# hahnyuan/PTQ4ViT

Hardware: AMD Instinct MI355X
Metric: calibration throughput (wrapped modules calibrated per second), ViT-B/224 W8A8, 32 calibration images (higher is better)
Workload: dtype int8

## Files before the change

include/ptq4vit_hip_debug.h:

```cpp
#ifndef PTQ4VIT_HIP_DEBUG_H
#define PTQ4VIT_HIP_DEBUG_H

#include <stddef.h>
#include <stdint.h>

#ifdef __cplusplus
extern "C" {
#endif

int p4v_debug_set_variant(int variant, int force_generic);
int p4v_debug_set_tuning(int key, int value);
int p4v_debug_bound_totals(float* out, int64_t capacity, int64_t* count);
int p4v_debug_set_arena_gap(size_t bytes);
int p4v_debug_arena_ranges(uint64_t* out, int cap);
int p4v_debug_mlp_planes(uint64_t* out);
int p4v_debug_attn_planes(uint64_t info[5]);
int p4v_debug_sos_sweep(const p4v_matmul_desc* desc, const float* d_A, const float* d_B, const float* d_out, const float* d_grad,
                        int n_cands, int c_lo, int c_hi, int known_cands, float* d_scores, void* d_workspace, size_t workspace_bytes,
                        void* stream);
int p4v_debug_topk_rows(const float* d_mass, int segs, int n, int k, int32_t* d_idx, void* stream);
int p4v_debug_pack_dual(const float* d_x, long rows, long cols, long cols_padded, int sos, int lo, int hi, int qmax,
                        const float* d_scale, float const_scale, int8_t* d_q1, int8_t* d_q2, void* stream);
int p4v_debug_pack_cands(const float* d_x, long rows, long cols, long rows_padded, long cols_padded, int layout, int lo, int hi,
                         const float* d_scales, int n_cands, const int* d_crange, const unsigned char* d_done, int live_max,
                         int general, int8_t* d_q, void* stream);
int p4v_debug_gather_im2col(int batch, int in_channels, int height, int width, int kernel_h, int kernel_w, int stride_h, int stride_w,
                            int pad_h, int pad_w, int dil_h, int dil_w, const float* d_x, const int32_t* d_idx, int k, float* d_dst,
                            void* stream);
int p4v_debug_prep_epi6(const float* d_o, const float* d_wt, const float* d_bias, long o_ss, long o_ts, int sr, int tr,
                        int bias_on_t, int wt_mode, int transposed, float* d_e, void* stream);

#ifdef __cplusplus
}
#endif
#endif
```

ptq4vit_amd/_lib.py:

```python
import ctypes as C
import os

_HERE = os.path.dirname(os.path.abspath(__file__))
LIB_PATH = os.environ.get("P4V_LIB") or os.path.join(_HERE, "csrc", "libptq4vit_hip.so")

METRICS = {
    "L1_norm": 0,
    "L2_norm": 1,
    "linear_weighted_L2_norm": 2,
    "square_weighted_L2_norm": 3,
    "hessian": 4,
    "cosine": 5,
}


class LinearDesc(C.Structure):
    _fields_ = [(n, C.c_int32) for n in (
        "batch", "tokens", "in_features", "out_features", "n_V", "n_H", "n_a", "w_bit", "a_bit", "metric",
        "eq_n", "search_round", "twin_postgelu", "init_layerwise", "has_bias", "reserved")]


class MlpDesc(C.Structure):
    _fields_ = [("fc1", LinearDesc), ("fc2", LinearDesc)]

# ... 63 lines not shown

JOB_LINEAR, JOB_MATMUL, JOB_CONV, JOB_MATMUL_BLOCKS = 0, 1, 2, 3
RESERVED_FP32_PLANES, RESERVED_NO_MEMO, RESERVED_FORWARD_ONLY, RESERVED_NO_PRUNE = 1, 2, 4, 8
RESERVED_BLOCK_SHIFT = 8


def reserved_block(block):
    return 0 if block is None else (int(block) + 1) << RESERVED_BLOCK_SHIFT


PLANE_SYM, PLANE_SOS_HI, PLANE_SOS_LO, PLANE_TWIN = 1, 2, 3, 4
EXPORT_SYM_I8, EXPORT_SYM_F32, EXPORT_GELU_U8, EXPORT_SOS_U8 = 0, 1, 2, 3


EXPORTS = [
    "p4v_version", "p4v_last_error",
    "p4v_linear_workspace_bytes", "p4v_linear_calibrate",
    "p4v_matmul_workspace_bytes", "p4v_matmul_calibrate",
    "p4v_matmul_blocks_workspace_bytes", "p4v_matmul_blocks_calibrate", "p4v_amax_init_matmul_blocks",
    "p4v_matmul_blocks_search", "p4v_matmul_blocks_quant_forward",
    "p4v_conv_workspace_bytes", "p4v_conv_calibrate",
    "p4v_calibrate_group", "p4v_launch_counters",
    "p4v_linear_quant_forward", "p4v_matmul_quant_forward", "p4v_mlp_workspace_bytes", "p4v_mlp_quant_forward",
    "p4v_attn_workspace_bytes", "p4v_attn_quant_forward",
    "p4v_amax_init_linear", "p4v_linear_search_w", "p4v_linear_search_a",
    "p4v_amax_init_matmul", "p4v_matmul_search_A", "p4v_sos_search_split", "p4v_matmul_search_B",
    "p4v_amax_init_conv", "p4v_conv_search_w_channelwise", "p4v_conv_search_w_layerwise", "p4v_conv_search_a",
    "p4v_score_argmax_gather",
    "p4v_quantize_i8", "p4v_pack_plane_i8", "p4v_fake_quant", "p4v_export_quantize", "p4v_multi_copy",
    "p4v_stats_enable", "p4v_stats_reset", "p4v_stats_get", "p4v_stats_launches", "p4v_prune_counters",
    "p4v_debug_set_variant", "p4v_debug_set_tuning", "p4v_debug_bound_totals", "p4v_debug_topk_rows", "p4v_debug_pack_dual", "p4v_debug_prep_epi6",
    "p4v_debug_pack_cands", "p4v_debug_gather_im2col", "p4v_debug_sos_sweep",
    "p4v_debug_set_arena_gap", "p4v_debug_arena_ranges", "p4v_debug_mlp_planes", "p4v_debug_attn_planes",
]

_lib = None


def load():
    global _lib
    if _lib is not None:
        return _lib
    if not os.path.exists(LIB_PATH):
        raise RuntimeError(
            f"ptq4vit_amd: HIP extension {LIB_PATH} is missing -- build it with "
            "`python -c 'import __graft_entry__ as g; g.build()'` (hipcc --offload-arch=gfx950). "
            "There is no CPU fallback for the calibration path.")
    import torch
    lib = C.CDLL(LIB_PATH)
    vp, fp, ip = C.c_void_p, C.c_void_p, C.c_void_p
    lib.p4v_version.restype = C.c_int
    lib.p4v_last_error.restype = C.c_char_p
    lib.p4v_linear_workspace_bytes.restype = C.c_size_t
    lib.p4v_linear_workspace_bytes.argtypes = [C.POINTER(LinearDesc)]
    lib.p4v_linear_calibrate.restype = C.c_int
    lib.p4v_linear_calibrate.argtypes = [C.POINTER(LinearDesc), fp, fp, fp, fp, fp, fp, fp, fp, fp, ip, vp, C.c_size_t, vp]
    lib.p4v_matmul_workspace_bytes.restype = C.c_size_t
    lib.p4v_matmul_workspace_bytes.argtypes = [C.POINTER(MatMulDesc)]
    lib.p4v_matmul_calibrate.restype = C.c_int
    lib.p4v_matmul_calibrate.argtypes = [C.POINTER(MatMulDesc), fp, fp, fp, fp, fp, fp, fp, fp, fp, ip, vp, C.c_size_t, vp]
    MBD = C.POINTER(MatMulBlocksDesc)
    lib.p4v_matmul_blocks_workspace_bytes.restype = C.c_size_t
    lib.p4v_matmul_blocks_workspace_bytes.argtypes = [MBD]
    lib.p4v_matmul_blocks_calibrate.restype = C.c_int
    lib.p4v_matmul_blocks_calibrate.argtypes = [MBD, fp, fp, fp, fp, fp, fp, fp, fp, fp, ip, vp, C.c_size_t, vp]
    lib.p4v_amax_init_matmul_blocks.restype = C.c_int
# ... 23 lines not shown
    lib.p4v_matmul_quant_forward.restype = C.c_int
    lib.p4v_matmul_quant_forward.argtypes = [C.POINTER(MatMulDesc), fp, fp, fp, fp, fp, fp, vp, C.c_size_t, vp]
    LD, MD, CD = C.POINTER(LinearDesc), C.POINTER(MatMulDesc), C.POINTER(ConvDesc)
    tail = [vp, C.c_size_t, vp]
    for name, args in (
            ("p4v_amax_init_linear", [LD] + [fp] * 4),
            ("p4v_linear_search_w", [LD] + [fp] * 9 + [ip]),
            ("p4v_linear_search_a", [LD] + [fp] * 9 + [ip]),
            ("p4v_amax_init_matmul", [MD] + [fp] * 4),
            ("p4v_matmul_search_A", [MD] + [fp] * 8 + [ip]),
            ("p4v_sos_search_split", [MD] + [fp] * 7 + [ip]),
            ("p4v_matmul_search_B", [MD] + [fp] * 9 + [ip]),
            ("p4v_amax_init_conv", [CD] + [fp] * 4),
            ("p4v_conv_search_w_channelwise", [CD] + [fp] * 9 + [ip]),
            ("p4v_conv_search_w_layerwise", [CD] + [fp] * 9 + [ip]),
            ("p4v_conv_search_a", [CD] + [fp] * 9 + [ip])):
        fn = getattr(lib, name)
        fn.restype = C.c_int
        fn.argtypes = args + tail
    lib.p4v_score_argmax_gather.restype = C.c_int
    lib.p4v_score_argmax_gather.argtypes = [fp, C.c_int32, C.c_int32, fp, fp, ip, vp]
    lib.p4v_quantize_i8.restype = C.c_int
    lib.p4v_quantize_i8.argtypes = [fp, C.c_int64, C.c_int64, C.c_int64, fp, C.c_int64, C.c_int32, C.c_int32, vp, vp]
    lib.p4v_fake_quant.restype = C.c_int
    lib.p4v_fake_quant.argtypes = [fp, C.c_int64, C.c_int64, fp, C.c_int64, C.c_int32, C.c_int32, fp, vp]
    lib.p4v_pack_plane_i8.restype = C.c_int
    lib.p4v_pack_plane_i8.argtypes = [C.POINTER(PlaneDesc), fp, fp, vp, vp]
    lib.p4v_export_quantize.restype = C.c_int
    lib.p4v_export_quantize.argtypes = [C.POINTER(ExportDesc), fp, fp, fp, vp, vp]
    lib.p4v_multi_copy.restype = C.c_int
    lib.p4v_multi_copy.argtypes = [vp, C.c_int32, C.c_int64, C.c_int64, vp]
    lib.p4v_debug_topk_rows.restype = C.c_int
    lib.p4v_debug_topk_rows.argtypes = [vp, C.c_int, C.c_int, C.c_int, vp, vp]
    lib.p4v_debug_pack_dual.restype = C.c_int
    lib.p4v_debug_pack_dual.argtypes = [fp, C.c_long, C.c_long, C.c_long, C.c_int, C.c_int, C.c_int, C.c_int, fp, C.c_float, vp, vp, vp]
    lib.p4v_debug_pack_cands.restype = C.c_int
    lib.p4v_debug_pack_cands.argtypes = [fp, C.c_long, C.c_long, C.c_long, C.c_long, C.c_int, C.c_int, C.c_int, fp, C.c_int, vp, vp,
                                         C.c_int, C.c_int, vp, vp]
    lib.p4v_debug_gather_im2col.restype = C.c_int
    lib.p4v_debug_gather_im2col.argtypes = [C.c_int] * 12 + [fp, ip, C.c_int, fp, vp]
    lib.p4v_debug_sos_sweep.restype = C.c_int
    lib.p4v_debug_sos_sweep.argtypes = [C.POINTER(MatMulDesc), fp, fp, fp, fp, C.c_int, C.c_int, C.c_int, C.c_int, fp, vp, C.c_size_t, vp]
    lib.p4v_debug_prep_epi6.restype = C.c_int
    lib.p4v_debug_prep_epi6.argtypes = [fp, fp, fp, C.c_long, C.c_long, C.c_int, C.c_int, C.c_int, C.c_int, C.c_int, fp, vp]
    lib.p4v_debug_set_variant.restype = C.c_int
    lib.p4v_debug_set_variant.argtypes = [C.c_int, C.c_int]
    lib.p4v_debug_set_tuning.restype = C.c_int
    lib.p4v_debug_set_tuning.argtypes = [C.c_int, C.c_int]
    lib.p4v_debug_set_arena_gap.restype = C.c_int
    lib.p4v_debug_set_arena_gap.argtypes = [C.c_size_t]
    lib.p4v_debug_arena_ranges.restype = C.c_int
    lib.p4v_debug_arena_ranges.argtypes = [C.POINTER(C.c_uint64), C.c_int]
    lib.p4v_debug_bound_totals.restype = C.c_int
    lib.p4v_debug_bound_totals.argtypes = [fp, C.c_int64, C.POINTER(C.c_int64)]
    lib.p4v_stats_enable.restype = C.c_int
    lib.p4v_stats_enable.argtypes = [C.c_int]
    lib.p4v_stats_reset.restype = C.c_int
    lib.p4v_stats_get.restype = C.c_int
    lib.p4v_stats_get.argtypes = [C.POINTER(KernelStats)]
    lib.p4v_stats_launches.restype = C.c_int
    lib.p4v_stats_launches.argtypes = [C.POINTER(LaunchRecord), C.c_int64, C.POINTER(C.c_int64)]
    lib.p4v_prune_counters.restype = C.c_int
    lib.p4v_prune_counters.argtypes = [C.POINTER(C.c_int64), C.c_int]
    lib.p4v_launch_counters.restype = C.c_int
    lib.p4v_launch_counters.argtypes = [C.POINTER(C.c_int64), C.c_int]
    lib.p4v_calibrate_group.restype = C.c_int
# ... 22 lines not shown
```

ptq4vit_amd/csrc/p4v_api.hip:

```cpp
#include <hip/hip_runtime.h>

#include <algorithm>
#include <atomic>
#include <climits>
#include <cstdarg>
#include <cstdio>
#include <condition_variable>
#include <cstring>
#include <deque>
#include <functional>
#include <thread>
#include <mutex>
#include <string>
#include <unordered_map>
#include <type_traits>
#include <vector>

#include "../../include/ptq4vit_hip.h"
#include "../../include/ptq4vit_hip_debug.h"
#include "p4v_kernels.h"

using namespace p4v;

namespace {
// ... 429 lines not shown
    for (auto& m : g_mir) if (m.dev == dev) return &m;
    return nullptr;
}
void attach_mirror(SelectParams& sl) {
    sl.iv_host = nullptr; sl.aux_host = nullptr;
    IvMirror* mi = mirror_of(sl.interval);
    IvMirror* ma = mirror_of(sl.aux_out);
    if (mi) mi->valid = false;
    if (ma) ma->valid = false;
    if (mi && sl.nj <= MIR_SLOT && sl.out_off == 0 && (sl.nj == 1 || sl.out_js == 1)) { sl.iv_host = mi->host; mi->valid = true; mi->count = sl.nj; }
    if (ma && sl.nj <= MIR_SLOT) { sl.aux_host = ma->host; ma->valid = true; ma->count = sl.nj; }
}

void metric_epi(int metric, int* epi, int* wt_mode) {
    switch (metric) {
        case P4V_METRIC_L1_NORM: *epi = EPI_ABS; *wt_mode = 0; break;
        case P4V_METRIC_L2_NORM: *epi = EPI_SQ; *wt_mode = 0; break;
        case P4V_METRIC_LINEAR_WEIGHTED_L2: *epi = EPI_W_SQ; *wt_mode = 3; break;
        case P4V_METRIC_SQUARE_WEIGHTED_L2: *epi = EPI_SQ_W; *wt_mode = 2; break;
        case P4V_METRIC_HESSIAN: *epi = EPI_SQ_W; *wt_mode = 1; break;
        default: *epi = EPI_COS; *wt_mode = 0; break;
    }
}

int launch_absmax(Ctx& c, const float* src, const long (&st)[4], int D0, int D1, int R, int C, int nV, int nH,
                  int crb_r, int crb_c, int signed_max, unsigned* out) {
    if (c.dry) return 0;
    CHK(q_fill(c, out, 0, sizeof(unsigned) * (size_t)D1 * nV * nH));
    AbsMaxParams p{src, st[0], st[1], st[2], st[3], D0, D1, R, C, nV, nH, crb_r, crb_c, 0, signed_max, out};
    p.row_tile = std::max(1, std::min(crb_r, std::max(1, 8192 / std::max(1, std::min(crb_c, C)))));
    const int tiles_per_v = cdiv(crb_r, p.row_tile);
    dim3 grid(tiles_per_v * nV * nH, D1, D0);
    return enqueue(c, KERN(AbsMaxParams, k_absmax), grid, dim3(256), 0, p);
}

int launch_interval(Ctx& c, const unsigned* enc, int n, float denom, int broadcast, float* interval) {
    if (c.dry) return 0;
    return enqueue(c, KERN(IntervalParams, k_interval_from_max), dim3(cdiv(n, 64)), dim3(64), 0, IntervalParams{enc, n, denom, broadcast, interval});
}

int launch_cands(Ctx& c, const float* mult, const float* interval, int ncand, int nblk, float* cands) {
    if (c.dry) return 0;
    return enqueue(c, KERN(CandsParams, k_make_cands), dim3(cdiv((long)ncand * nblk, 256)), dim3(256), 0, CandsParams{mult, interval, ncand, nblk, cands});
}

int launch_scale(Ctx& c, ScaleParams p) {
    if (c.dry) return 0;
    return enqueue(c, KERN(ScaleParams, k_scale_table), dim3(cdiv((long)p.C * p.nblk, 256)), dim3(256), 0, p);
}

std::atomic<int> g_cvt_state{0};
void cvt_probe(hipStream_t stream) {
    if (g_cvt_state.load(std::memory_order_acquire) != 0) return;
    static std::mutex mu;
    std::lock_guard<std::mutex> lk(mu);
    if (g_cvt_state.load(std::memory_order_acquire) != 0) return;
    static unsigned* scratch = nullptr;
    if (!scratch && hipMalloc(&scratch, 8 * sizeof(unsigned)) != hipSuccess) { (void)hipGetLastError(); scratch = nullptr; return; }
    unsigned h[5] = {9, 9, 9, 9, 9};
    hipLaunchKernelGGL(k_probe_cvt, dim3(1), dim3(64), 0, stream, scratch);
    if (hipGetLastError() != hipSuccess || hipMemcpyAsync(h, scratch, sizeof h, hipMemcpyDeviceToHost, stream) != hipSuccess ||
        hipStreamSynchronize(stream) != hipSuccess) { (void)hipGetLastError(); return; }
    const bool sat = h[3] == 0 && h[4] == 255;
    const int st = (sat && h[0] == 0 && h[1] == 1 && h[2] == 2) ? 1 : (sat && h[0] == 1 && h[1] == 2 && (h[2] == 2 || h[2] == 3)) ? 2 : 3;
    if (tune(TUNE_PRINT) > 0) fprintf(stderr, "[p4v] v_cvt_pk_u8_f32(0.7, 1.5, 2.5, -3, 300) = %u %u %u %u %u -> mode %d\n", h[0], h[1], h[2], h[3], h[4], st);
    g_cvt_state.store(st, std::memory_order_release);
// ... 679 lines not shown

int pack_operand(Ctx& c, const Pass& ps, const SweepPlan& pl, const PassBufs& b, const Operand& op, char* buf, bool col, int c0, int nc) {
    PackParams pk = op.pk;
    pk.Rp = col ? pl.NpB : pl.Mp; pk.Kp = pl.Kp; pk.dst = buf;
    pk.Z = (col ? ps.col_zs_shared : ps.row_zs_shared) ? 1 : ps.Z;
    pk.C = op.expanded ? nc : 1;
    pk.c_inner = op.expanded ? pl.cin_exp : pl.cin_fix;
    if (op.expanded && pk.scales) pk.scales += (long)c0 * pk.sc_cs;
    if (op.expanded && ps.crange) {
        pk.crange = ps.crange; pk.c_base = c0;
        pk.done = (b.pc && b.pc->done) ? b.pc->done : nullptr;
    }
    int live_max = -1;
    if (pk.crange && ps.host_hi > ps.host_lo) live_max = std::max(0, std::min(ps.host_hi, c0 + nc) - std::max(ps.host_lo, c0));
    else if (pk.crange && ps.host_len > 0) live_max = std::min(ps.host_len, nc);
    return ps.i8 ? launch_pack<int8_t>(c, pk, live_max) : launch_pack<float>(c, pk, live_max);
}
int pack_expanded(Ctx& c, const Pass& ps, const SweepPlan& pl, const PassBufs& b, int c0, int nc) {
    PlaneCache* pc = b.pc;
    const bool packed = pc && pc->valid;
    if (ps.row.expanded && !packed) CHK(pack_operand(c, ps, pl, b, ps.row, b.row, false, c0, nc));
    if (ps.twin && ps.row2.expanded) CHK(pack_operand(c, ps, pl, b, ps.row2, b.row2, false, c0, nc));
    if (ps.col.expanded && !packed) CHK(pack_operand(c, ps, pl, b, ps.col, b.col, true, c0, nc));
    if (pc && !ps.crange && !packed) {
        pc->valid = true;
        if (!c.dry && pc->done) CHK(q_fill(c, pc->done, 1, (size_t)ps.eq_n));
    }
    return 0;
}

int prep_epilogue(Ctx& c, const Pass& ps, const SweepPlan& pl, const PassBufs& b) {
    const bool a_search = pl.a_search;
    const size_t zero_bytes = sizeof(float) * pl.zero_bias_n;
    if (pl.epi6_on && !c.dry && !(b.ec && b.ec->valid)) {
        PrepEpi6Params pe{};
        pe.O = ps.O; pe.Wt = ps.G ? ps.G : ps.O; pe.bias = ps.bias ? ps.bias : b.zero_bias;
        pe.o_ss = a_search ? ps.o_ns : ps.o_ms; pe.o_ts = a_search ? ps.o_ms : ps.o_ns;
        pe.SR = a_search ? ps.Ncols : ps.Mrows; pe.TR = a_search ? ps.Mrows : ps.Ncols;
        pe.bias_on_t = a_search ? 0 : 1; pe.wt_mode = ps.cos6 ? 4 : ps.wt_mode;
        pe.stiles = pl.s6_stiles; pe.ttiles = pl.s6_ttiles; pe.E = b.epi6; pe.transposed = (ps.cos6 && !a_search) ? 1 : 0;
        if (b.zero_bias) CHK(q_fill(c, b.zero_bias, 0, zero_bytes));
        CHK(enqueue(c, KERN(PrepEpi6Params, k_prep_epi6), dim3((unsigned)std::min<long>((long)pl.s6_stiles * pl.s6_ttiles, 256L * 32)), dim3(256), 0, pe));
    }
    if (b.ec) b.ec->valid = true;
    if (pl.epi7_n && !c.dry) {
        PrepEpiParams pe{ps.O, ps.G ? ps.G : ps.O, ps.bias, ps.o_ms, ps.Mrows, ps.Ncols, ps.cos7 ? 4 : ps.wt_mode,
                         pl.Np / 256, pl.Mp / (ps.twin ? 128 : 256), ps.twin ? 1 : 0, b.epi7};
        const long chunks = (long)pl.Mp * pl.Np * 2 / 4;
        CHK(enqueue(c, KERN(PrepEpiParams, k_prep_epi), dim3((unsigned)std::min<long>(cdiv(chunks, 256), 256L * 16)), dim3(256), 0, pe));
    }
    if (b.zero_bias && !c.dry) CHK(q_fill(c, b.zero_bias, 0, zero_bytes));
    return 0;
}

int pack_fixed_planes(Ctx& c, const Pass& ps, const SweepPlan& pl, const PassBufs& b) {
    if (ps.row.prepacked) {
        if (ps.row.expanded || pl.merged7 || pl.cin_fix != 0 || (ps.twin && (!ps.row2.prepacked || ps.row2.expanded)))
            return fail(P4V_ERR_INVALID, "prepacked row operand: fixed row-major plane(s) of a forward pass only");
    } else if (pl.merged7) {
        Operand both = ps.row;
        both.pk.mode = PACK_TWIN_I8;
        both.pk.lo = ps.row2.pk.lo; both.pk.neg_scale = ps.row2.pk.neg_scale;
        both.pk.dst2 = b.row2;
        CHK(pack_operand(c, ps, pl, b, both, b.row, false, 0, 1));
    } else if (ps.twin && ps.i8 && !ps.row.expanded && !ps.row2.expanded && dual_pack_ok(ps.row.pk, ps.row2.pk)) {
        PackParams p1 = ps.row.pk, p2 = ps.row2.pk;
        p1.Rp = p2.Rp = pl.Mp; p1.Kp = p2.Kp = pl.Kp; p1.Z = p2.Z = ps.row_zs_shared ? 1 : ps.Z; p1.C = p2.C = 1;
        p1.dst = b.row; p2.dst = b.row2;
        if (!c.dry) {
            const long total = (long)p1.Z * pl.Mp * (pl.Kp / 16);
            if (total >= (1L << 31)) return fail(P4V_ERR_UNSUPPORTED, "operand plane too large for k_pack_dual (%ld 16-element runs)", total);
            CHK(enqueue(c, KERN(PackDualParams, k_pack_dual), dim3((unsigned)std::min<long>(cdiv(total, 256), 256L * 64)), dim3(256), 0, PackDualParams{p1, p2}));
        }
    } else {
        if (!ps.row.expanded) CHK(pack_operand(c, ps, pl, b, ps.row, b.row, false, 0, 1));
        if (ps.twin && !ps.row2.expanded) CHK(pack_operand(c, ps, pl, b, ps.row2, b.row2, false, 0, 1));
    }
    if (!ps.col.expanded) CHK(pack_operand(c, ps, pl, b, ps.col, b.col, true, 0, 1));
    return 0;
}

int chunk_exec_frac(Ctx& c, const Pass& ps, const SweepPlan& pl, int c0, int nc) {
    g_exec_frac = 1.0;
    if (!(g_stat_on && ps.crange && !c.dry)) return 0;
// ... 213 lines not shown
    bool conv; PackParams conv_pk;
    int k_cap;
};
int slice_alloc(Ctx& c, SliceCache* sc, const SliceGeo& g, bool keep, bool bump) {
    if (sc->assigned) {
        if (sc->k != g.k_cap) return fail(P4V_ERR_INVALID, "slice cache reused with another geometry");
        return 0;
    }
    if (!keep && !bump) return 0;
    const long zrows = (long)g.segs * g.seg_rows, out_elems = (long)g.segs * g.k_cap * g.Ncols, row_elems = (long)g.segs * g.k_cap * g.K;
    if (keep) {
        sc->idx = reinterpret_cast<int*>(c.ws.get_top((size_t)g.segs * g.k_cap * sizeof(int)));
        sc->mass = reinterpret_cast<float*>(c.ws.get_top((size_t)zrows * sizeof(float)));
        sc->Os = reinterpret_cast<float*>(c.ws.get_top((size_t)out_elems * sizeof(float)));
        sc->Gs = reinterpret_cast<float*>(c.ws.get_top((size_t)out_elems * sizeof(float)));
        sc->Rs = reinterpret_cast<float*>(c.ws.get_top((size_t)row_elems * sizeof(float)));
        sc->frac = reinterpret_cast<float*>(c.ws.get_top(256));
        sc->assigned = true;
    } else {
        sc->idx = c.ws.get<int>((size_t)g.segs * g.k_cap);
        sc->mass = c.ws.get<float>((size_t)zrows);
        sc->Os = c.ws.get<float>((size_t)out_elems);
        sc->Gs = c.ws.get<float>((size_t)out_elems);
        sc->Rs = c.ws.get<float>((size_t)row_elems);
    }
    sc->k = g.k_cap;
    return 0;
}
int slice_fill(Ctx& c, SliceCache* sc, const SliceGeo& g, bool host_sync_ok) {
    const long zrows = (long)g.segs * g.seg_rows;
    const void* wsrc = g.G ? (const void*)g.G : (const void*)g.O;
    const bool new_idx = sc->idx_src != wsrc || sc->idx_wt != g.wt_mode || (g.wt_mode != 1 && sc->o_src != g.O);
    if (new_idx) {
        CHK(enqueue(c, KERN(RowMassParams, k_row_mass), dim3((unsigned)cdiv(zrows, 4)), dim3(256), 0, RowMassParams{g.G ? g.G : g.O, g.O, zrows, (long)g.Ncols, g.wt_mode, sc->mass}));
        CHK(enqueue(c, KERN(TopkParams, k_topk_rows), dim3(g.segs), dim3(1024), 0, TopkParams{sc->mass, g.seg_rows, g.k, sc->idx}));
        sc->idx_src = wsrc; sc->idx_wt = g.wt_mode;
        sc->o_src = sc->g_src = sc->r_src = nullptr;
        if (sc->frac && host_sync_ok && !(g_variant & 8388608)) {
            float f = 1.0f;
            int* hm = host_mirror(c);
            CHK(enqueue(c, KERN(MassFracParams, k_mass_fraction), dim3(1), dim3(1024), 0,
                        MassFracParams{sc->mass, zrows, sc->idx, g.segs, g.seg_rows, g.k, sc->frac, hm ? reinterpret_cast<float*>(hm + 4) : nullptr}));
            if (!hm) CHK(q_d2h(c, &f, sc->frac, sizeof f));
            CHK(q_sync(c));
            if (hm) f = *reinterpret_cast<volatile float*>(hm + 4);
            if (tune(TUNE_PRINT) > 0) fprintf(stderr, "[p4v] slice holds %.4f of the metric weight (%d x %d of %d rows)\n", f, g.segs, g.k, g.seg_rows);
            sc->frac_host = f;
            if (g.k < g.k_cap && !(f >= 0.97f)) {
                SliceGeo g2 = g;
                g2.k = g.k_cap;
                sc->idx_src = nullptr;
                return slice_fill(c, sc, g2, host_sync_ok);
            }
            const bool big_pass = zrows >= (tune(TUNE_LOOSE_ROWS) > 0 ? (long)tune(TUNE_LOOSE_ROWS) : 65536L);
            if (!(f >= (tune(TUNE_LOOSE_PCT) > 0 ? 0.01f * tune(TUNE_LOOSE_PCT) : big_pass ? 0.05f : 0.5f))) { sc->loose = true; return 0; }
        }
        sc->k_eff = g.k;
    }
    const int rows = g.segs * g.k;
    int gather_rc = 0;
    auto gather = [&](const float* src, long s0, long s3, int d3, float* dst, int seg, int zdiv, long sz2, long sz) {
        GatherParams gp{src, s0, 0, 0, s3, 1, 1, d3, sc->idx, rows, dst, seg, zdiv, sz2, sz};
        const long total = (long)rows * d3;
        if (const int r_ = enqueue(c, KERN(GatherParams, k_gather), dim3((unsigned)std::min<long>(cdiv(total, 256), 256L * 16)), dim3(256), 0, gp)) gather_rc = r_;
    };
    const int seg = g.lin ? 0 : g.k;
    const long o_seg = (long)g.seg_rows * g.Ncols;
// ... 2267 lines not shown
int p4v_debug_sos_sweep(const p4v_matmul_desc* desc, const float* d_A, const float* d_B, const float* d_out, const float* d_grad,
                        int n_cands, int c_lo, int c_hi, int known_cands, float* d_scores, void* d_workspace, size_t workspace_bytes,
                        void* stream) {
    if (!desc || !d_A || !d_B || !d_out || !d_scores || !d_workspace) return fail(P4V_ERR_INVALID, "p4v_debug_sos_sweep: null pointer");
    if (!desc->sos || n_cands < 1 || n_cands > 20 || !sos_split_ok(desc->M, desc->K, desc->N, false))
        return fail(P4V_ERR_INVALID, "p4v_debug_sos_sweep: a split-of-softmax matmul of the one-kernel split search, 1..20 candidates");
    const SosDebugSweep dbg{n_cands, c_lo, c_hi, known_cands, d_scores};
    float* d_split = nullptr;
    CHK(ws_aligned(d_workspace));
    HIPCHK(hipMalloc(&d_split, 2 * sizeof(float)));
    Ctx c = Ctx::on(stream, d_workspace, workspace_bytes);
    g_sos_debug = &dbg;
    const int rc = matmul_impl(desc, {.A = d_A, .B = d_B, .O = d_out, .G = d_grad, .A_iv = d_split + 1, .split = d_split}, Stage{ST_S1}, c);
    g_sos_debug = nullptr;
    (void)hipFree(d_split);
    return rc;
}

int p4v_debug_bound_totals(float* out, int64_t capacity, int64_t* count) {
    if (!out && !count) { g_b1_keep = true; g_b1_totals.clear(); return 0; }
    g_b1_keep = false;
    if (count) *count = (int64_t)g_b1_totals.size();
    if (out) std::copy(g_b1_totals.begin(), g_b1_totals.begin() + std::min<int64_t>(capacity, (int64_t)g_b1_totals.size()), out);
    return 0;
}

int p4v_debug_topk_rows(const float* d_mass, int segs, int n, int k, int32_t* d_idx, void* stream) {
    if (!d_mass || !d_idx || segs <= 0 || n <= 0 || k <= 0 || k > n) return fail(P4V_ERR_INVALID, "p4v_debug_topk_rows: bad argument");
    hipLaunchKernelGGL(k_topk_rows, dim3(segs), dim3(1024), 0, (hipStream_t)stream, TopkParams{d_mass, n, k, d_idx});
    HIPCHK(hipGetLastError());
    return 0;
}

int p4v_debug_pack_dual(const float* d_x, long rows, long cols, long cols_padded, int sos, int lo, int hi, int qmax,
                        const float* d_scale, float const_scale, int8_t* d_q1, int8_t* d_q2, void* stream) {
    if (!d_x || !d_scale || !d_q1 || !d_q2 || rows <= 0 || cols <= 0 || cols_padded % 64 || cols_padded < cols ||
        lo > 0 || hi < 0 || lo < -128 || hi > 127 || qmax < 2 || qmax > 128 || (!sos && !(const_scale > 0.0f)))
        return fail(P4V_ERR_INVALID, "p4v_debug_pack_dual: bad argument");
    PackParams p1 = pack2d(d_x, rows, cols, cols);
    p1.Rp = (int)rows; p1.Kp = (int)cols_padded; p1.C = 1; p1.scales = d_scale; p1.qm1 = (float)(qmax - 1);
    PackParams p2 = p1;
    p1.dst = d_q1; p2.dst = d_q2;
    if (sos) {
        p1.mode = PACK_SOS_HI; p2.mode = PACK_SOS_LO;
    } else {
        p1.lo = 0; p1.hi = hi; p2.lo = lo; p2.hi = 0; p2.scales = nullptr; p2.neg_scale = const_scale;
    }
    if (!dual_pack_ok(p1, p2)) return fail(P4V_ERR_INVALID, "p4v_debug_pack_dual: not a dual pair");
    Ctx c = Ctx::on(stream, nullptr, 0);
    const long total = rows * (cols_padded / 16);
    if (total >= (1L << 31)) return fail(P4V_ERR_UNSUPPORTED, "p4v_debug_pack_dual: plane too large");
    return enqueue(c, KERN(PackDualParams, k_pack_dual), dim3((unsigned)std::min<long>(cdiv(total, 256), 256L * 64)), dim3(256), 0,
                   PackDualParams{p1, p2});
}

int p4v_debug_pack_cands(const float* d_x, long rows, long cols, long rows_padded, long cols_padded, int layout, int lo, int hi,
                         const float* d_scales, int n_cands, const int* d_crange, const unsigned char* d_done, int live_max,
                         int general, int8_t* d_q, void* stream) {
    if (!d_x || !d_scales || !d_q || rows <= 0 || cols <= 0 || rows_padded < rows || cols_padded % 64 || cols_padded < cols ||
        layout < 0 || layout > 3 || (layout == 3 && rows_padded % 64) || lo > hi || lo < -128 || hi > 127 || n_cands <= 0 ||
        (d_done && !d_crange) || (live_max >= 0 && !d_crange))
        return fail(P4V_ERR_INVALID, "p4v_debug_pack_cands: bad argument");
    Ctx c = Ctx::on(stream, nullptr, 0);
    cvt_bias(c);
    PackParams p = pack2d(d_x, rows, cols, cols);
    p.Rp = (int)rows_padded; p.Kp = (int)cols_padded; p.dst = d_q; p.C = n_cands; p.c_inner = layout;
// ... 96 lines not shown
```

ptq4vit_amd/csrc/p4v_kernels.h:

```cpp
#pragma once
#include <hip/hip_runtime.h>
#include <stdint.h>
#include <type_traits>

namespace p4v {

typedef int v4i __attribute__((ext_vector_type(4)));
typedef int v16i __attribute__((ext_vector_type(16)));
typedef float v4f __attribute__((ext_vector_type(4)));
typedef float v16f __attribute__((ext_vector_type(16)));
typedef float v2f __attribute__((ext_vector_type(2)));

#ifndef P4V_GROUP_KERNARG
#define P4V_GROUP_KERNARG (4096 - 256)
#endif
template <typename P> struct GroupArgs {
    static constexpr int CAP_RAW = (P4V_GROUP_KERNARG - 16) / (int)(sizeof(P) + 16);
    static constexpr int CAP = CAP_RAW > 64 ? 64 : CAP_RAW;
    int n;
    unsigned off[CAP + 1];
    unsigned gx[CAP], gy[CAP], gz[CAP];
    P p[CAP];
};
#define P4V_BIDX uint3{blockIdx.x, blockIdx.y, blockIdx.z}
#define P4V_GDIM uint3{gridDim.x, gridDim.y, gridDim.z}
#define P4V_GROUP_ENTER(a)                                                                           \
    int m_ = 0;                                                                                      \
    while (m_ + 1 < a.n && blockIdx.x >= a.off[m_ + 1]) ++m_;                                        \
    m_ = __builtin_amdgcn_readfirstlane(m_);                                                         \
    const unsigned b_ = blockIdx.x - a.off[m_];                                                      \
    const uint3 vg_{a.gx[m_], a.gy[m_], a.gz[m_]};                                                   \
    if (b_ >= vg_.x * vg_.y * vg_.z) return;                                                         \
    const uint3 vb_{b_ % vg_.x, (b_ / vg_.x) % vg_.y, b_ / (vg_.x * vg_.y)}

__device__ __forceinline__ unsigned enc_ordered(float f) {
    unsigned b = __float_as_uint(f);
    return (b & 0x80000000u) ? ~b : (b | 0x80000000u);
}
__device__ __forceinline__ float dec_ordered(unsigned e) {
    unsigned b = (e & 0x80000000u) ? (e & 0x7fffffffu) : ~e;
    return __uint_as_float(b);
}

struct AbsMaxParams {
    const float* src;
    long s0, s1, s2, s3;
    int D0, D1, R, C;
    int nV, nH, crb_r, crb_c;
    int row_tile;
    int signed_max;
    unsigned* out;
};

__device__ __forceinline__ void k_absmax_body(const AbsMaxParams& p, const uint3 blockIdx, const uint3 gridDim) {
    int bx = blockIdx.x;
    const int h = bx % p.nH; bx /= p.nH;
    const int v = bx % p.nV; bx /= p.nV;
    const int rt = bx;
    const int r0 = v * p.crb_r + rt * p.row_tile;
    const int r1 = min(min(r0 + p.row_tile, (v + 1) * p.crb_r), p.R);
    const int c0 = h * p.crb_c;
    const int c1 = min(c0 + p.crb_c, p.C);
    const int w = c1 - c0;
    const float* base = p.src + (long)blockIdx.z * p.s0 + (long)blockIdx.y * p.s1;
    float m = -INFINITY;
    if (w > 0 && r1 > r0 && p.s3 == 1 && (w & 3) == 0 && (p.s2 & 3) == 0 && (c0 & 3) == 0 && ((((unsigned long long)base) & 15) == 0)) {
        const int w4 = w >> 2;
        const int tpr = w4 >= 256 ? 256 : w4 >= 128 ? 128 : w4 >= 64 ? 64 : w4 >= 32 ? 32 : 16;
        const int tx = threadIdx.x & (tpr - 1), ty = threadIdx.x / tpr, rpar = 256 / tpr;
        for (int r = r0 + ty; r < r1; r += rpar) {
            const v4f* row = reinterpret_cast<const v4f*>(base + (long)r * p.s2 + c0);
            for (int c = tx; c < w4; c += tpr) {
                const v4f x = row[c];
                if (p.signed_max) m = fmaxf(fmaxf(m, fmaxf(x[0], x[1])), fmaxf(x[2], x[3]));
                else m = fmaxf(fmaxf(m, fmaxf(fabsf(x[0]), fabsf(x[1]))), fmaxf(fabsf(x[2]), fabsf(x[3])));
            }
        }
    } else if (w > 0 && r1 > r0) {
        const int n = (r1 - r0) * w;
        for (int i = threadIdx.x; i < n; i += 256) {
            const int r = r0 + i / w, c = c0 + i % w;
            float x = base[(long)r * p.s2 + (long)c * p.s3];
            m = fmaxf(m, p.signed_max ? x : fabsf(x));
        }
    }
    for (int o = 32; o > 0; o >>= 1) m = fmaxf(m, __shfl_xor(m, o));
    __shared__ float red[4];
    if ((threadIdx.x & 63) == 0) red[threadIdx.x >> 6] = m;
    __syncthreads();
    if (threadIdx.x == 0) {
        m = fmaxf(fmaxf(red[0], red[1]), fmaxf(red[2], red[3]));
        if (m > -INFINITY) atomicMax(p.out + ((long)blockIdx.y * p.nV + v) * p.nH + h, enc_ordered(m));
    }
}
__global__ __launch_bounds__(256) void k_absmax(AbsMaxParams p) { k_absmax_body(p, P4V_BIDX, P4V_GDIM); }
__global__ __launch_bounds__(256) void k_absmax_g(GroupArgs<AbsMaxParams> a) { P4V_GROUP_ENTER(a); k_absmax_body(a.p[m_], vb_, vg_); }

struct IntervalParams { const unsigned* enc; int n; float denom; int broadcast; float* interval; };
__device__ __forceinline__ void k_interval_from_max_body(const IntervalParams& a, const uint3 blockIdx, const uint3 gridDim) {
    const auto& [enc, n, denom, broadcast, interval] = a;
    int j = blockIdx.x * blockDim.x + threadIdx.x;
    if (j >= n) return;
    float m;
    if (broadcast) {
        m = -INFINITY;
        for (int i = 0; i < n; ++i) m = fmaxf(m, dec_ordered(enc[i]));
    } else {
        m = dec_ordered(enc[j]);
    }
    interval[j] = m / denom;
// ... 3570 lines not shown
    const int c = blockIdx.x, j = blockIdx.y, nt = blockDim.x;
    double acc = 0.0;
    if (p.j_mode == 3) {
        const int smp = j * nt + threadIdx.x;
        if (smp < p.S) {
            for (int zb = 0; zb < p.ZB; ++zb) acc += (double)cos_item(p, c, zb, 0, p.ZV, smp);
            p.scores[(long)c * p.nj + smp] = (float)(p.norm * acc);
        }
        return;
    }
    int zv0 = 0, zv1 = p.ZV, zlo = 0, zstep = 1;
    if (p.j_mode == 1) { zv0 = j; zv1 = j + 1; }
    if (p.j_mode == 2) { zlo = j; zstep = p.j_div; }
    const int nz = (p.ZB - zlo + zstep - 1) / zstep;
    const long total = (long)nz * p.S;
    for (long i = threadIdx.x; i < total; i += nt) {
        const int smp = (int)(i % p.S);
        const int zb = zlo + (int)(i / p.S) * zstep;
        acc += (double)cos_item(p, c, zb, zv0, zv1, smp);
    }
    __shared__ double red[1024];
    red[threadIdx.x] = acc;
    __syncthreads();
    for (int o = nt >> 1; o > 0; o >>= 1) {
        if (threadIdx.x < o) red[threadIdx.x] += red[threadIdx.x + o];
        __syncthreads();
    }
    if (threadIdx.x == 0) p.scores[(long)c * p.nj + j] = (float)(p.norm * red[0]);
}
__global__ __launch_bounds__(1024) void k_finish_cos(FinishCosParams p) { k_finish_cos_body(p, P4V_BIDX, P4V_GDIM); }
__global__ __launch_bounds__(1024) void k_finish_cos_g(GroupArgs<FinishCosParams> a) { P4V_GROUP_ENTER(a); k_finish_cos_body(a.p[m_], vb_, vg_); }

struct RowMassParams { const float* W; const float* O; long rows; long cols; int wt_mode; float* mass; };
__device__ __forceinline__ void k_row_mass_body(const RowMassParams& a_, const uint3 blockIdx, const uint3 gridDim) {
    const auto& [W, O, rows, cols, wt_mode, mass] = a_;
    const long r = (long)blockIdx.x * 4 + (threadIdx.x >> 6);
    if (r >= rows) return;
    const int lane = threadIdx.x & 63;
    const float* src = (wt_mode == 1 ? W : O) + r * cols;
    float s = 0.0f;
    if (wt_mode == 0) s = lane == 0 ? 1.0f : 0.0f;
    else
        for (long i = lane; i < cols; i += 64) {
            const float v = src[i];
            s += wt_mode == 2 ? fabsf(v) : v * v;
        }
    for (int o = 32; o > 0; o >>= 1) s += __shfl_xor(s, o);
    if (lane == 0) mass[r] = s;
}
__global__ __launch_bounds__(256) void k_row_mass(RowMassParams p) { k_row_mass_body(p, P4V_BIDX, P4V_GDIM); }
__global__ __launch_bounds__(256) void k_row_mass_g(GroupArgs<RowMassParams> a) { P4V_GROUP_ENTER(a); k_row_mass_body(a.p[m_], vb_, vg_); }
__global__ void k_group_mass(const float* mass, int n_groups, int group, float* out) {
    const int g = blockIdx.x * blockDim.x + threadIdx.x;
    if (g >= n_groups) return;
    float s = 0.0f;
    for (int i = 0; i < group; ++i) s += mass[(long)g * group + i];
    out[g] = s;
}
struct TopkParams { const float* mass_all; int n; int k; int* idx_all; };
__device__ __forceinline__ void k_topk_rows_body(const TopkParams& a_, const uint3 blockIdx, const uint3 gridDim) {
    const auto& [mass_all, n, k, idx_all] = a_;
    const float* mass = mass_all + (long)blockIdx.x * n;
    int* idx = idx_all + (long)blockIdx.x * k;
    __shared__ int hist[256];
    __shared__ int wtot[4];
    __shared__ int wg[2][16], we[2][16];
    __shared__ unsigned prefix_s;
    __shared__ int krem_s;
    const int t = threadIdx.x, lane = t & 63, wv = t >> 6;
    auto key = [&](int i) -> unsigned { const unsigned b = __float_as_uint(mass[i]); return (b & 0x80000000u) ? 0u : b; };
    if (t == 0) { prefix_s = 0; krem_s = k; }
    for (int shift = 24; shift >= 0; shift -= 8) {
        if (t < 256) hist[t] = 0;
        __syncthreads();
        const unsigned hi_mask = shift == 24 ? 0u : (0xFFFFFFFFu << (shift + 8));
        const unsigned pre = prefix_s;
        const int kr = krem_s;
        for (int i0 = 0; i0 < n; i0 += 1024) {
            const int i = i0 + t;
            const unsigned kv = i < n ? key(i) : 0u;
            const bool in = i < n && (kv & hi_mask) == pre;
// ... 757 lines not shown
```

ptq4vit_amd/engine.py:

```python
import ctypes as C

import torch

from . import _lib

_workspace = {}
_mult_cache = {}


def _require_cuda(t, what):
    if not t.is_cuda:
        raise RuntimeError(f"ptq4vit_amd: {what} must live on the GPU (got {t.device}); the calibration path has no CPU fallback")


def device_of(*tensors):
    for t in tensors:
        if t is not None and t.is_cuda:
            return t.device
    if not torch.cuda.is_available():
        raise RuntimeError("ptq4vit_amd: no GPU visible -- the HIP calibration engine needs an MI355X (no CPU fallback)")
    return torch.device("cuda", torch.cuda.current_device())


def to_dev(t, dev):
# ... 704 lines not shown
    _lib.check(_lib.load().p4v_debug_set_arena_gap(int(nbytes)), "p4v_debug_set_arena_gap")


def debug_arena_ranges():
    lib = _lib.load()
    n = lib.p4v_debug_arena_ranges(None, 0)
    buf = (C.c_uint64 * max(2, 2 * n))()
    n = min(n, lib.p4v_debug_arena_ranges(buf, n))
    return [(int(buf[2 * i]), int(buf[2 * i + 1])) for i in range(n)]


def debug_bound_totals(start=False):
    lib = _lib.load()
    if start:
        _lib.check(lib.p4v_debug_bound_totals(None, 0, None), "p4v_debug_bound_totals")
        return None
    n = C.c_int64(0)
    _lib.check(lib.p4v_debug_bound_totals(None, 0, C.byref(n)), "p4v_debug_bound_totals")
    buf = (C.c_float * max(1, n.value))()
    _lib.check(lib.p4v_debug_bound_totals(buf, n.value, C.byref(n)), "p4v_debug_bound_totals")
    return [float(v) for v in buf[:n.value]]


def debug_topk_rows(mass, k):
    assert mass.is_cuda and mass.dtype == torch.float32 and mass.dim() == 2 and mass.is_contiguous()
    segs, n = mass.shape
    out = torch.empty(segs, int(k), dtype=torch.int32, device=mass.device)
    with torch.cuda.device(mass.device):
        rc = _lib.load().p4v_debug_topk_rows(ptr(mass), segs, n, int(k), ptr(out), stream_ptr(mass.device))
    _lib.check(rc, "p4v_debug_topk_rows")
    return out


def debug_pack_dual(x2d, *, sos, scale, lo, hi, qmax, const_scale=0.0):
    x2d = x2d.contiguous().float()
    rows, cols = x2d.shape
    colsp = (cols + 63) // 64 * 64
    q1 = torch.empty(rows, colsp, dtype=torch.int8, device=x2d.device)
    q2 = torch.empty_like(q1)
    sc = torch.tensor([float(scale)], dtype=torch.float32, device=x2d.device)
    with torch.cuda.device(x2d.device):
        rc = _lib.load().p4v_debug_pack_dual(ptr(x2d), rows, cols, colsp, int(bool(sos)), int(lo), int(hi), int(qmax), ptr(sc),
                                             float(const_scale), ptr(q1), ptr(q2), stream_ptr(x2d.device))
    _lib.check(rc, "p4v_debug_pack_dual")
    return q1[:, :cols], q2[:, :cols], q1, q2


def debug_pack_cands(x2d, scales, *, layout, lo, hi, rows_padded=None, crange=None, done=None, live_max=-1, general=False,
                     out=None):
    x2d = x2d.contiguous().float()
    scales = scales.contiguous().float()
    rows, cols = x2d.shape
    n = scales.numel()
    colsp = (cols + 63) // 64 * 64
    rowsp = rows if rows_padded is None else int(rows_padded)
    size = rowsp * colsp * (1 if layout == 3 else (n + 1) // 2 * 2 if layout == 2 else n)
    if out is None:
        out = torch.zeros(size, dtype=torch.int8, device=x2d.device)
    assert out.dtype == torch.int8 and out.is_contiguous() and out.numel() >= size
    with torch.cuda.device(x2d.device):
        rc = _lib.load().p4v_debug_pack_cands(ptr(x2d), rows, cols, rowsp, colsp, int(layout), int(lo), int(hi), ptr(scales), n,
                                              ptr(crange) if crange is not None else None,
                                              ptr(done) if done is not None else None, int(live_max), int(bool(general)),
                                              ptr(out), stream_ptr(x2d.device))
    _lib.check(rc, "p4v_debug_pack_cands")
    return out
# ... 71 lines not shown
```

Baseline: 687.2.

## Rework absmax and row-mass kernels with unrolled loads and multi-row waves

Rewrites the absmax reduction kernel to flatten each tile into a linear vector-load index space, unrolled eight deep, with separate handling for unaligned head and tail elements. This lets unaligned or odd-width tiles use vectorised loads instead of the scalar fallback. Rewrites the row-mass kernel so each wave handles several short rows at once and unrolls loads for long rows. It also stops filling the zero-bias buffer twice in the epilogue prep, and adds debug entry points for both kernels. The new edge and NaN-padding logic is intricate and could mishandle boundary cases.

After: 693.4, median of 4. About the same (+0.9%).

```diff
diff --git a/include/ptq4vit_hip_debug.h b/include/ptq4vit_hip_debug.h
--- a/include/ptq4vit_hip_debug.h
+++ b/include/ptq4vit_hip_debug.h
@@ -19,6 +19,9 @@
                         int n_cands, int c_lo, int c_hi, int known_cands, float* d_scores, void* d_workspace, size_t workspace_bytes,
                         void* stream);
 int p4v_debug_topk_rows(const float* d_mass, int segs, int n, int k, int32_t* d_idx, void* stream);
+int p4v_debug_row_mass(const float* d_w, const float* d_o, long rows, long cols, int wt_mode, float* d_mass, void* stream);
+int p4v_debug_absmax(const float* d_src, const int64_t* stride, const int32_t* dims, int nV, int nH, int signed_max, uint32_t* d_enc,
+                     void* stream);
 int p4v_debug_pack_dual(const float* d_x, long rows, long cols, long cols_padded, int sos, int lo, int hi, int qmax,
                         const float* d_scale, float const_scale, int8_t* d_q1, int8_t* d_q2, void* stream);
 int p4v_debug_pack_cands(const float* d_x, long rows, long cols, long rows_padded, long cols_padded, int layout, int lo, int hi,
diff --git a/ptq4vit_amd/_lib.py b/ptq4vit_amd/_lib.py
--- a/ptq4vit_amd/_lib.py
+++ b/ptq4vit_amd/_lib.py
@@ -119,6 +119,7 @@
     "p4v_debug_set_variant", "p4v_debug_set_tuning", "p4v_debug_bound_totals", "p4v_debug_topk_rows", "p4v_debug_pack_dual", "p4v_debug_prep_epi6",
     "p4v_debug_pack_cands", "p4v_debug_gather_im2col", "p4v_debug_sos_sweep",
     "p4v_debug_set_arena_gap", "p4v_debug_arena_ranges", "p4v_debug_mlp_planes", "p4v_debug_attn_planes",
+    "p4v_debug_row_mass", "p4v_debug_absmax",
 ]
 
 _lib = None
@@ -208,6 +209,11 @@
     lib.p4v_multi_copy.argtypes = [vp, C.c_int32, C.c_int64, C.c_int64, vp]
     lib.p4v_debug_topk_rows.restype = C.c_int
     lib.p4v_debug_topk_rows.argtypes = [vp, C.c_int, C.c_int, C.c_int, vp, vp]
+    if hasattr(lib, "p4v_debug_row_mass"):
+        lib.p4v_debug_row_mass.restype = C.c_int
+        lib.p4v_debug_row_mass.argtypes = [fp, fp, C.c_long, C.c_long, C.c_int, fp, vp]
+        lib.p4v_debug_absmax.restype = C.c_int
+        lib.p4v_debug_absmax.argtypes = [fp, C.POINTER(C.c_int64), C.POINTER(C.c_int32), C.c_int, C.c_int, C.c_int, vp, vp]
     lib.p4v_debug_pack_dual.restype = C.c_int
     lib.p4v_debug_pack_dual.argtypes = [fp, C.c_long, C.c_long, C.c_long, C.c_int, C.c_int, C.c_int, C.c_int, fp, C.c_float, vp, vp, vp]
     lib.p4v_debug_pack_cands.restype = C.c_int
diff --git a/ptq4vit_amd/csrc/p4v_api.hip b/ptq4vit_amd/csrc/p4v_api.hip
--- a/ptq4vit_amd/csrc/p4v_api.hip
+++ b/ptq4vit_amd/csrc/p4v_api.hip
@@ -485,6 +485,11 @@
     const int tiles_per_v = cdiv(crb_r, p.row_tile);
     dim3 grid(tiles_per_v * nV * nH, D1, D0);
     return enqueue(c, KERN(AbsMaxParams, k_absmax), grid, dim3(256), 0, p);
+}
+
+int launch_row_mass(Ctx& c, const RowMassParams& p) {
+    if (c.dry) return 0;
+    return enqueue(c, KERN(RowMassParams, k_row_mass), dim3((unsigned)cdiv(p.rows, 4L * row_mass_rows_per_wave(p.cols))), dim3(256), 0, p);
 }
 
 int launch_interval(Ctx& c, const unsigned* enc, int n, float denom, int broadcast, float* interval) {
@@ -1230,6 +1235,7 @@
 int prep_epilogue(Ctx& c, const Pass& ps, const SweepPlan& pl, const PassBufs& b) {
     const bool a_search = pl.a_search;
     const size_t zero_bytes = sizeof(float) * pl.zero_bias_n;
+    bool zero_filled = false;
     if (pl.epi6_on && !c.dry && !(b.ec && b.ec->valid)) {
         PrepEpi6Params pe{};
         pe.O = ps.O; pe.Wt = ps.G ? ps.G : ps.O; pe.bias = ps.bias ? ps.bias : b.zero_bias;
@@ -1237,7 +1243,7 @@
         pe.SR = a_search ? ps.Ncols : ps.Mrows; pe.TR = a_search ? ps.Mrows : ps.Ncols;
         pe.bias_on_t = a_search ? 0 : 1; pe.wt_mode = ps.cos6 ? 4 : ps.wt_mode;
         pe.stiles = pl.s6_stiles; pe.ttiles = pl.s6_ttiles; pe.E = b.epi6; pe.transposed = (ps.cos6 && !a_search) ? 1 : 0;
-        if (b.zero_bias) CHK(q_fill(c, b.zero_bias, 0, zero_bytes));
+        if (b.zero_bias) { CHK(q_fill(c, b.zero_bias, 0, zero_bytes)); zero_filled = true; }
         CHK(enqueue(c, KERN(PrepEpi6Params, k_prep_epi6), dim3((unsigned)std::min<long>((long)pl.s6_stiles * pl.s6_ttiles, 256L * 32)), dim3(256), 0, pe));
     }
     if (b.ec) b.ec->valid = true;
@@ -1247,7 +1253,7 @@
         const long chunks = (long)pl.Mp * pl.Np * 2 / 4;
         CHK(enqueue(c, KERN(PrepEpiParams, k_prep_epi), dim3((unsigned)std::min<long>(cdiv(chunks, 256), 256L * 16)), dim3(256), 0, pe));
     }
-    if (b.zero_bias && !c.dry) CHK(q_fill(c, b.zero_bias, 0, zero_bytes));
+    if (b.zero_bias && !c.dry && !zero_filled) CHK(q_fill(c, b.zero_bias, 0, zero_bytes));
     return 0;
 }
 
@@ -1527,7 +1533,7 @@
     const void* wsrc = g.G ? (const void*)g.G : (const void*)g.O;
     const bool new_idx = sc->idx_src != wsrc || sc->idx_wt != g.wt_mode || (g.wt_mode != 1 && sc->o_src != g.O);
     if (new_idx) {
-        CHK(enqueue(c, KERN(RowMassParams, k_row_mass), dim3((unsigned)cdiv(zrows, 4)), dim3(256), 0, RowMassParams{g.G ? g.G : g.O, g.O, zrows, (long)g.Ncols, g.wt_mode, sc->mass}));
+        CHK(launch_row_mass(c, RowMassParams{g.G ? g.G : g.O, g.O, zrows, (long)g.Ncols, g.wt_mode, sc->mass}));
         CHK(enqueue(c, KERN(TopkParams, k_topk_rows), dim3(g.segs), dim3(1024), 0, TopkParams{sc->mass, g.seg_rows, g.k, sc->idx}));
         sc->idx_src = wsrc; sc->idx_wt = g.wt_mode;
         sc->o_src = sc->g_src = sc->r_src = nullptr;
@@ -3861,6 +3867,22 @@
     return 0;
 }
 
+int p4v_debug_row_mass(const float* d_w, const float* d_o, long rows, long cols, int wt_mode, float* d_mass, void* stream) {
+    if (!d_o || !d_mass || rows <= 0 || cols <= 0 || wt_mode < 0 || wt_mode > 3 || (wt_mode == 1 && !d_w))
+        return fail(P4V_ERR_INVALID, "p4v_debug_row_mass: bad argument");
+    Ctx c = Ctx::on(stream, nullptr, 0);
+    return launch_row_mass(c, RowMassParams{d_w ? d_w : d_o, d_o, rows, cols, wt_mode, d_mass});
+}
+
+int p4v_debug_absmax(const float* d_src, const int64_t* stride, const int32_t* dims, int nV, int nH, int signed_max, uint32_t* d_enc,
+                     void* stream) {
+    if (!d_src || !stride || !dims || !d_enc || nV <= 0 || nH <= 0 || dims[0] <= 0 || dims[1] <= 0 || dims[2] <= 0 || dims[3] <= 0)
+        return fail(P4V_ERR_INVALID, "p4v_debug_absmax: bad argument");
+    Ctx c = Ctx::on(stream, nullptr, 0);
+    const long st[4] = {(long)stride[0], (long)stride[1], (long)stride[2], (long)stride[3]};
+    return launch_absmax(c, d_src, st, dims[0], dims[1], dims[2], dims[3], nV, nH, cdiv(dims[2], nV), cdiv(dims[3], nH), signed_max ? 1 : 0, d_enc);
+}
+
 int p4v_debug_pack_dual(const float* d_x, long rows, long cols, long cols_padded, int sos, int lo, int hi, int qmax,
                         const float* d_scale, float const_scale, int8_t* d_q1, int8_t* d_q2, void* stream) {
     if (!d_x || !d_scale || !d_q1 || !d_q2 || rows <= 0 || cols <= 0 || cols_padded % 64 || cols_padded < cols ||
diff --git a/ptq4vit_amd/csrc/p4v_kernels.h b/ptq4vit_amd/csrc/p4v_kernels.h
--- a/ptq4vit_amd/csrc/p4v_kernels.h
+++ b/ptq4vit_amd/csrc/p4v_kernels.h
@@ -52,6 +52,7 @@
     unsigned* out;
 };
 
+constexpr int ABSMAX_U = 8;
 __device__ __forceinline__ void k_absmax_body(const AbsMaxParams& p, const uint3 blockIdx, const uint3 gridDim) {
     int bx = blockIdx.x;
     const int h = bx % p.nH; bx /= p.nH;
@@ -64,18 +65,52 @@
     const int w = c1 - c0;
     const float* base = p.src + (long)blockIdx.z * p.s0 + (long)blockIdx.y * p.s1;
     float m = -INFINITY;
-    if (w > 0 && r1 > r0 && p.s3 == 1 && (w & 3) == 0 && (p.s2 & 3) == 0 && (c0 & 3) == 0 && ((((unsigned long long)base) & 15) == 0)) {
-        const int w4 = w >> 2;
-        const int tpr = w4 >= 256 ? 256 : w4 >= 128 ? 128 : w4 >= 64 ? 64 : w4 >= 32 ? 32 : 16;
-        const int tx = threadIdx.x & (tpr - 1), ty = threadIdx.x / tpr, rpar = 256 / tpr;
-        for (int r = r0 + ty; r < r1; r += rpar) {
-            const v4f* row = reinterpret_cast<const v4f*>(base + (long)r * p.s2 + c0);
-            for (int c = tx; c < w4; c += tpr) {
-                const v4f x = row[c];
-                if (p.signed_max) m = fmaxf(fmaxf(m, fmaxf(x[0], x[1])), fmaxf(x[2], x[3]));
-                else m = fmaxf(fmaxf(m, fmaxf(fabsf(x[0]), fabsf(x[1]))), fmaxf(fabsf(x[2]), fabsf(x[3])));
-            }
-        }
+    if (w > 0 && r1 > r0 && p.s3 == 1) {
+        constexpr int U = ABSMAX_U;
+        const float* tile = base + (long)r0 * p.s2 + c0;
+        const bool aligned = (p.s2 & 3) == 0 && ((unsigned long long)tile & 15) == 0;
+        const int nrows = r1 - r0;
+        const int nv = aligned ? w >> 2 : (w + 3) >> 2;
+        const int total = nrows * nv;
+        const float qnan = __builtin_nanf("");
+        auto edge = [&](int i) -> float {
+            const int row = i / 6, j = i - row * 6;
+            const float* rp = tile + (long)row * p.s2;
+            const int head = min((int)((0 - ((unsigned long long)rp >> 2)) & 3), w);
+            const int e = j < 3 ? j : head + ((w - head) & ~3) + (j - 3);
+            return (row < nrows && (j < 3 ? e < head : e < w)) ? rp[e] : qnan;
+        };
+        const bool edges = !aligned || (w & 3) != 0;
+        float xe = edges ? edge(threadIdx.x) : qnan;
+        if (nv > 0) {
+            const int dr = 256 / nv, dk = 256 % nv;
+            for (int i0 = threadIdx.x; i0 < total; i0 += 256 * U) {
+                v4f x[U];
+                int row = i0 / nv, k = i0 - row * nv;
+#pragma unroll
+                for (int u = 0; u < U; ++u) {
+                    x[u] = v4f{qnan, qnan, qnan, qnan};
+                    if (i0 + 256 * u < total) {
+                        const float* rp = tile + (long)row * p.s2;
+                        const int e0 = 4 * k - (aligned ? 0 : (int)(((unsigned long long)rp >> 2) & 3));
+                        if (e0 >= 0 && e0 + 4 <= w) x[u] = *reinterpret_cast<const v4f*>(rp + e0);
+                    }
+                    k += dk; row += dr;
+                    if (k >= nv) { k -= nv; ++row; }
+                }
+#pragma unroll
+                for (int u = 0; u < U; ++u) {
+                    if (p.signed_max) m = fmaxf(fmaxf(m, fmaxf(x[u][0], x[u][1])), fmaxf(x[u][2], x[u][3]));
+                    else m = fmaxf(fmaxf(m, fmaxf(fabsf(x[u][0]), fabsf(x[u][1]))), fmaxf(fabsf(x[u][2]), fabsf(x[u][3])));
+                }
+            }
+        }
+        m = fmaxf(m, p.signed_max ? xe : fabsf(xe));
+        if (edges)
+            for (int i = threadIdx.x + 256; i < nrows * 6; i += 256) {
+                xe = edge(i);
+                m = fmaxf(m, p.signed_max ? xe : fabsf(xe));
+            }
     } else if (w > 0 && r1 > r0) {
         const int n = (r1 - r0) * w;
         for (int i = threadIdx.x; i < n; i += 256) {
@@ -3712,21 +3747,74 @@
 __global__ __launch_bounds__(1024) void k_finish_cos_g(GroupArgs<FinishCosParams> a) { P4V_GROUP_ENTER(a); k_finish_cos_body(a.p[m_], vb_, vg_); }
 
 struct RowMassParams { const float* W; const float* O; long rows; long cols; int wt_mode; float* mass; };
+constexpr int ROW_MASS_U = 8;
+__host__ __device__ inline int row_mass_rows_per_wave(long cols) { return cols <= 64 ? 16 : cols <= 128 ? 8 : cols <= 256 ? 4 : 1; }
+template <bool ABS> __device__ __forceinline__ float row_mass_add(float s, float v) {
+#pragma clang fp contract(off)
+    const float t = ABS ? fabsf(v) : v * v;
+    return s + t;
+}
+template <bool ABS> __device__ __forceinline__ void row_mass_long(const float* src, long cols, int lane, float* mass) {
+    constexpr int U = ROW_MASS_U;
+    float s = 0.0f;
+    for (long b = 0; b < cols; b += 64 * U) {
+        float v[U];
+        if (b + 64 * U <= cols) {
+#pragma unroll
+            for (int u = 0; u < U; ++u) v[u] = src[b + 64 * u + lane];
+#pragma unroll
+            for (int u = 0; u < U; ++u) s = row_mass_add<ABS>(s, v[u]);
+        } else {
+#pragma unroll
+            for (int u = 0; u < U; ++u) v[u] = src[min(b + 64 * u + lane, cols - 1)];
+#pragma unroll
+            for (int u = 0; u < U; ++u)
+                if (b + 64 * u + lane < cols) s = row_mass_add<ABS>(s, v[u]);
+        }
+    }
+    for (int o = 32; o > 0; o >>= 1) s += __shfl_xor(s, o);
+    if (lane == 0) *mass = s;
+}
+template <int CH, int RW, bool ABS>
+__device__ __forceinline__ void row_mass_short(const float* src, long rows, long cols, long r, int lane, float* mass) {
+    float v[RW][CH], s[RW];
+#pragma unroll
+    for (int q = 0; q < RW; ++q) {
+        const float* row = src + min(r + q, rows - 1) * cols;
+#pragma unroll
+        for (int j = 0; j < CH; ++j) v[q][j] = row[min((long)(64 * j + lane), cols - 1)];
+    }
+#pragma unroll
+    for (int q = 0; q < RW; ++q) {
+        s[q] = 0.0f;
+#pragma unroll
+        for (int j = 0; j < CH; ++j)
+            if (64 * j + lane < cols) s[q] = row_mass_add<ABS>(s[q], v[q][j]);
+    }
+    for (int o = 32; o > 0; o >>= 1) {
+#pragma unroll
+        for (int q = 0; q < RW; ++q) s[q] += __shfl_xor(s[q], o);
+    }
+    float out = s[0];
+#pragma unroll
+    for (int q = 1; q < RW; ++q) out = lane == q ? s[q] : out;
+    if (lane < RW && r + lane < rows) mass[r + lane] = out;
+}
 __device__ __forceinline__ void k_row_mass_body(const RowMassParams& a_, const uint3 blockIdx, const uint3 gridDim) {
     const auto& [W, O, rows, cols, wt_mode, mass] = a_;
-    const long r = (long)blockIdx.x * 4 + (threadIdx.x >> 6);
+    const int lane = threadIdx.x & 63;
+    const long r = ((long)blockIdx.x * 4 + (threadIdx.x >> 6)) * row_mass_rows_per_wave(cols);
     if (r >= rows) return;
-    const int lane = threadIdx.x & 63;
-    const float* src = (wt_mode == 1 ? W : O) + r * cols;
-    float s = 0.0f;
-    if (wt_mode == 0) s = lane == 0 ? 1.0f : 0.0f;
-    else
-        for (long i = lane; i < cols; i += 64) {
-            const float v = src[i];
-            s += wt_mode == 2 ? fabsf(v) : v * v;
-        }
-    for (int o = 32; o > 0; o >>= 1) s += __shfl_xor(s, o);
-    if (lane == 0) mass[r] = s;
+    if (wt_mode == 0) {
+        if (lane < row_mass_rows_per_wave(cols) && r + lane < rows) mass[r + lane] = 1.0f;
+        return;
+    }
+    const float* src = wt_mode == 1 ? W : O;
+    if (cols <= 64) { if (wt_mode == 2) row_mass_short<1, 16, true>(src, rows, cols, r, lane, mass); else row_mass_short<1, 16, false>(src, rows, cols, r, lane, mass); }
+    else if (cols <= 128) { if (wt_mode == 2) row_mass_short<2, 8, true>(src, rows, cols, r, lane, mass); else row_mass_short<2, 8, false>(src, rows, cols, r, lane, mass); }
+    else if (cols <= 256) { if (wt_mode == 2) row_mass_short<4, 4, true>(src, rows, cols, r, lane, mass); else row_mass_short<4, 4, false>(src, rows, cols, r, lane, mass); }
+    else if (wt_mode == 2) row_mass_long<true>(src + r * cols, cols, lane, mass + r);
+    else row_mass_long<false>(src + r * cols, cols, lane, mass + r);
 }
 __global__ __launch_bounds__(256) void k_row_mass(RowMassParams p) { k_row_mass_body(p, P4V_BIDX, P4V_GDIM); }
 __global__ __launch_bounds__(256) void k_row_mass_g(GroupArgs<RowMassParams> a) { P4V_GROUP_ENTER(a); k_row_mass_body(a.p[m_], vb_, vg_); }
diff --git a/ptq4vit_amd/engine.py b/ptq4vit_amd/engine.py
--- a/ptq4vit_amd/engine.py
+++ b/ptq4vit_amd/engine.py
@@ -760,6 +760,32 @@
     return out
 
 
+def debug_row_mass(o, w=None, *, wt_mode):
+    assert o.is_cuda and o.dtype == torch.float32 and o.dim() == 2 and o.is_contiguous()
+    assert w is None or (w.shape == o.shape and w.dtype == torch.float32 and w.is_contiguous() and w.device == o.device)
+    rows, cols = o.shape
+    mass = torch.empty(rows, dtype=torch.float32, device=o.device)
+    with torch.cuda.device(o.device):
+        rc = _lib.load().p4v_debug_row_mass(ptr(w) if w is not None else None, ptr(o), rows, cols, int(wt_mode), ptr(mass),
+                                            stream_ptr(o.device))
+    _lib.check(rc, "p4v_debug_row_mass")
+    return mass
+
+
+def debug_absmax(view, *, nV=1, nH=1, signed_max=False):
+    assert view.is_cuda and view.dtype == torch.float32 and view.dim() == 4
+    D1 = view.shape[1]
+    enc = torch.empty(D1, int(nV), int(nH), dtype=torch.int32, device=view.device)
+    st = (C.c_int64 * 4)(*view.stride())
+    dims = (C.c_int32 * 4)(*view.shape)
+    with torch.cuda.device(view.device):
+        rc = _lib.load().p4v_debug_absmax(view.data_ptr(), st, dims, int(nV), int(nH), int(bool(signed_max)), ptr(enc),
+                                          stream_ptr(view.device))
+    _lib.check(rc, "p4v_debug_absmax")
+    bits = torch.where(enc < 0, enc & 0x7fffffff, ~enc)
+    return bits.view(torch.float32), enc
+
+
 def debug_pack_dual(x2d, *, sos, scale, lo, hi, qmax, const_scale=0.0):
     x2d = x2d.contiguous().float()
     rows, cols = x2d.shape
```
